# ribal-aladeeb/reinforcement-learning-2048

Hardware: AMD Instinct MI355X
Metric: 2048 env steps/sec + DQN updates/sec at 64k parallel boards, 1→8 MI355X (higher is better)
Workload: dtype u8

## Files before the change

reinforcement-learning-2048_amd/csrc/g2048_learn64.hip:

```cpp
#include <hip/hip_runtime.h>
#include <math.h>
#include <stdint.h>
#include <stdlib.h>

#include "../../include/g2048.h"
#include "g2048_board.hpp"
#include "g2048_common.hpp"

namespace {

constexpr int NT = 256;
constexpr int S = 64;
constexpr int XS = 17;
constexpr int HS = 65;
constexpr int P_W1 = 0, P_B1 = 1024, P_W2 = 1088, P_B2 = 1344, P_N = 1348;
constexpr int SLAB = P_N + 4;
constexpr int MAX_SLABS = 256;

struct Net64 {
    double *w1, *b1, *w2, *b2;
};

struct alignas(16) Smem {
    double x[S * XS];
    double h[S * HS];
    double w2[2][4 * 64];
    double b1[2][64];
    double b2[2][4];
    double qa[S * 4];
    double qb[S * 4];
    double y[S];
    double dq[S];
    double loss[S];
    int act[S];
};

__device__ __forceinline__ int64_t sample_row(int64_t b, unsigned long long ep,
                                              unsigned long long count, uint32_t lo, uint32_t hi) {
    const uint4 u = g2048::philox10(
        make_uint4((uint32_t)b, (uint32_t)((uint64_t)b >> 32), (uint32_t)ep,
                   (uint32_t)(ep >> 32) | (g2048::DOMAIN_SAMPLE << 30)),
        lo, hi);
    return (int64_t)__umul64hi(((unsigned long long)u.y << 32) | u.x, count);
}

__device__ __forceinline__ void put_row(double* xr, uint4 v) {
    const uint32_t w[4] = {v.x, v.y, v.z, v.w};
#pragma unroll
    for (int k = 0; k < 4; ++k) {
        xr[4 * k + 0] = (double)(w[k] & 0xFFu);
        xr[4 * k + 1] = (double)((w[k] >> 8) & 0xFFu);
        xr[4 * k + 2] = (double)((w[k] >> 16) & 0xFFu);
        xr[4 * k + 3] = (double)(w[k] >> 24);
    }
}

__device__ __forceinline__ void forward(Smem& M, const double (&w1r)[16], int net, double* q) {
    const int t = threadIdx.x, j = t & 63, rq = t >> 6;
    const double bj = M.b1[net][j];
#pragma unroll 4
    for (int rr = 0; rr < 16; ++rr) {
        const int s = rq * 16 + rr;
        const double* xr = M.x + s * XS;
        double acc = 0.0;
#pragma unroll
        for (int k = 0; k < 16; ++k) acc = fma(w1r[k], xr[k], acc);
        const double pre = acc + bj;
        M.h[s * HS + j] = pre > 0.0 ? pre : 0.0;
    }
    __syncthreads();
    const int s = t >> 2, a = t & 3;
    const double* hr = M.h + s * HS;
    const double* w2 = M.w2[net] + a * 64;
    double acc = 0.0;
#pragma unroll 8
    for (int jj = 0; jj < 64; ++jj) acc = fma(w2[jj], hr[jj], acc);
    q[s * 4 + a] = acc + M.b2[net][a];
    __syncthreads();
}

struct UpdArgs64 {
    Net64 on, tg;
    const uint4 *s, *s2;
    const uint8_t *a, *d;
    const int32_t* r;
    const unsigned long long* count;
    const unsigned long long* step;
    const int64_t* idx_in;
    int64_t batch;
    uint32_t seed_lo, seed_hi;
    float gamma;
    int double_dqn;
    int64_t* idx_out;
    double* y_out;
    double* slab;
    unsigned long long* step_next;
};

typedef uint32_t u32x2 __attribute__((ext_vector_type(2)));
constexpr int AUX_SC1 = 16;
__device__ __forceinline__ __amdgpu_buffer_rsrc_t slab_rsrc(const double* base) {
    return __builtin_amdgcn_make_buffer_rsrc(const_cast<double*>(base), 0, 0x7FFFFFFF, 0x00020000);
}
template <bool COH>
__device__ __forceinline__ void slab_put(double* sl, int e, double v) {
    if constexpr (COH)
        __builtin_amdgcn_raw_buffer_store_b64(__builtin_bit_cast(u32x2, v), slab_rsrc(sl),
                                              (uint32_t)e * 8u, 0u, AUX_SC1);
    else
        sl[e] = v;
}

template <bool COH>
__device__ __forceinline__ void update_tiles64(const UpdArgs64& A) {
    __shared__ Smem M;
    const int t = threadIdx.x, j = t & 63, qd = t >> 6;
    const unsigned long long ep = A.idx_in ? 0ull : *A.step;
    const unsigned long long count = A.idx_in ? 0ull : *A.count;
    if (blockIdx.x == 0 && t == 0) *A.step_next = *A.step + 1ull;
    const Net64 nets[2] = {A.tg, A.on};
    double w1t[16], w1o[16];
#pragma unroll
    for (int k = 0; k < 16; ++k) {
        w1t[k] = A.tg.w1[j * 16 + k];
        w1o[k] = A.on.w1[j * 16 + k];
    }
    for (int i = t; i < 2 * 256; i += NT) M.w2[i >> 8][i & 255] = nets[i >> 8].w2[i & 255];
    if (t < 128) M.b1[t >> 6][t & 63] = nets[t >> 6].b1[t & 63];
    if (t < 8) M.b2[t >> 2][t & 3] = nets[t >> 2].b2[t & 3];
    double w2o[4];
#pragma unroll
    for (int a = 0; a < 4; ++a) w2o[a] = A.on.w2[a * 64 + j];
    double g_w1[4] = {0.0, 0.0, 0.0, 0.0}, g_b1 = 0.0, g_w2 = 0.0, g_b2 = 0.0, g_loss = 0.0;
    const int64_t ntiles = (A.batch + S - 1) / S;
    for (int64_t tile = blockIdx.x; tile < ntiles; tile += gridDim.x) {
        const int64_t b = tile * S + t;
        uint4 sv = make_uint4(0u, 0u, 0u, 0u);
        double rj = 0.0;
        float disc = 0.f;
        bool ok = false;
        __syncthreads();
        if (t < S) {
            uint4 s2v = make_uint4(0u, 0u, 0u, 0u);
            int aj = 0;
            ok = b < A.batch;
            if (ok) {
                const int64_t row =
                    A.idx_in ? A.idx_in[b] : sample_row(b, ep, count, A.seed_lo, A.seed_hi);
                A.idx_out[b] = row;
                s2v = A.s2[row];
                sv = A.s[row];
                aj = A.a[row];
                rj = (double)A.r[row];
                disc = (float)(1 - (int)A.d[row]) * A.gamma;
            }
            put_row(M.x + t * XS, s2v);
            M.act[t] = aj;
        }
        __syncthreads();
        forward(M, w1t, 0, M.qa);
        forward(M, w1o, 1, M.qb);
        if (t < S) {
            const double* qo = M.qb + t * 4;
            const double* qt = M.qa + t * 4;
            double next;
            if (A.double_dqn) {
                const uint32_t as = g2048::argmax4_torch(qo[0], qo[1], qo[2], qo[3]);
                next = qt[as];
            } else {
                next = g2048::qmax4_torch(qt[0], qt[1], qt[2], qt[3]);
            }
            double y;
            {
#pragma clang fp contract(off)
                y = rj + (double)disc * next;
            }
            M.y[t] = y;
            if (ok) A.y_out[b] = y;
            put_row(M.x + t * XS, sv);
        }
        __syncthreads();
        forward(M, w1o, 1, M.qb);
        if (t < S) {
            double dq = 0.0, l = 0.0;
            if (ok) {
#pragma clang fp contract(off)
                const double e = M.qb[t * 4 + M.act[t]] - M.y[t];
                dq = 2.0 * e;
                l = e * e;
            }
            M.dq[t] = dq;
            M.loss[t] = l;
        }
        __syncthreads();
        {
            double acc = 0.0, accb = 0.0;
            for (int s = 0; s < S; ++s) {
                if (M.act[s] == qd) {
                    acc = fma(M.dq[s], M.h[s * HS + j], acc);
                    accb += M.dq[s];
                }
            }
            g_w2 += acc;
            if (j == 0) g_b2 += accb;
        }
        if (t == 0) {
            double l = 0.0;
            for (int s = 0; s < S; ++s) l += M.loss[s];
            g_loss += l;
        }
        __syncthreads();
#pragma unroll 4
        for (int rr = 0; rr < 16; ++rr) {
            const int s = qd * 16 + rr;
            double& hv = M.h[s * HS + j];
            const double w = M.act[s] == 0 ? w2o[0] : M.act[s] == 1 ? w2o[1]
                           : M.act[s] == 2 ? w2o[2] : w2o[3];
            hv = hv > 0.0 ? M.dq[s] * w : 0.0;
        }
        __syncthreads();
        {
            double acc[4] = {0.0, 0.0, 0.0, 0.0}, accb = 0.0;
            for (int s = 0; s < S; ++s) {
                const double dh = M.h[s * HS + j];
                const double* xr = M.x + s * XS + 4 * qd;
#pragma unroll
                for (int i = 0; i < 4; ++i) acc[i] = fma(dh, xr[i], acc[i]);
                accb += dh;
            }
#pragma unroll
            for (int i = 0; i < 4; ++i) g_w1[i] += acc[i];
            if (qd == 0) g_b1 += accb;
        }
    }
    double* sl = A.slab + (int64_t)blockIdx.x * SLAB;
#pragma unroll
    for (int i = 0; i < 4; ++i) slab_put<COH>(sl, P_W1 + j * 16 + 4 * qd + i, g_w1[i]);
    if (qd == 0) slab_put<COH>(sl, P_B1 + j, g_b1);
    slab_put<COH>(sl, P_W2 + qd * 64 + j, g_w2);
    if (j == 0) slab_put<COH>(sl, P_B2 + qd, g_b2);
    if (t == 0) slab_put<COH>(sl, P_N, g_loss);
}

__global__ __launch_bounds__(NT) void k_dense64_update_f64(UpdArgs64 A) { update_tiles64<false>(A); }

constexpr int RW = 16;
static_assert(MAX_SLABS <= RW * 16, "reduction covers at most RW*16 slabs");

struct RedArgs64 {
    const double* slab;
    int nslab;
    double* grad;
    double* loss;
    const unsigned long long* step_next;
    unsigned long long* step;
    double* p[4];
    double* tp[4];
    unsigned long long sync_every;
    double* m;
    double* v;
    double lr, b1, b2, eps;
    int adam;
};

template <int NW, bool COH>
__device__ __forceinline__ void reduce_positions64(const RedArgs64& A, int chunk,
                                                   unsigned long long t, double (*part)[64]) {
    const int lane = threadIdx.x & 63, wave = threadIdx.x >> 6;
    const int pos = chunk * 64 + lane;
    const int k = pos < P_B1 ? 0 : pos < P_W2 ? 1 : pos < P_B2 ? 2 : 3;
    const int base[4] = {P_W1, P_B1, P_W2, P_B2};
    const bool adam = A.adam && wave == 0 && pos < P_N;
    double am = 0.0, av = 0.0, ap = 0.0;
    if (adam) {
// ... 195 lines not shown
```

reinforcement-learning-2048_amd/csrc/g2048_mlp.hip:

```cpp
#include <hip/hip_runtime.h>
#include <stdint.h>
#include <stdlib.h>

#include "../../include/g2048.h"
#include "g2048_board.hpp"
#include "g2048_common.hpp"

namespace {

constexpr int NT = 256, H = 64;
constexpr int XS = 20, W1S = 17, HS = 68, W2S = 68;
constexpr int S_FWD = 64;
constexpr int S_UPD = 32;
constexpr int P_W1 = 0, P_B1 = 1024, P_W2 = 1088, P_B2 = 1344, P_N = 1348;
constexpr int SLAB = 1352;
constexpr int MAX_SLABS = 256;

struct MlpW {
    const float *w1, *b1, *w2, *b2;
};

struct alignas(16) LW {
    float w1[H * W1S];
    float b1[H];
    float w2[4 * W2S];
    float b2[4];
};

template <int S>
struct alignas(16) Tile {
    float x[S * XS];
    float h[S * HS];
    float q[S * 4];
    float a[S], y[S], g[S];
};

__device__ __forceinline__ void stage_weights(const MlpW& W, LW& L) {
    const int t = threadIdx.x;
#pragma unroll
    for (int u = 0; u < 4; ++u) {
        const int e = u * NT + t;
        L.w1[(e >> 4) * W1S + (e & 15)] = W.w1[e];
    }
    if (t < H) L.b1[t] = W.b1[t];
    L.w2[(t >> 6) * W2S + (t & 63)] = W.w2[t];
    if (t < 4) L.b2[t] = W.b2[t];
// ... 62 lines not shown
            }
            T.h[s * HS + j] = fmaxf((p[0] + p[1]) + (p[2] + p[3]), 0.f);
        }
    }
    __syncthreads();
    layer2_tile<S>(T, W);
}

typedef float f32x4m __attribute__((ext_vector_type(4)));

__device__ __forceinline__ float4 w1_lane(const MlpW& W) {
    const int lane = threadIdx.x & 63, wave = threadIdx.x >> 6;
    return reinterpret_cast<const float4*>(W.w1)[(16 * wave + (lane & 15)) * 4 + (lane >> 4)];
}

template <int S>
__device__ __forceinline__ void forward_tile_mfma(Tile<S>& T, const LW& W, float4 w1v) {
    const int lane = threadIdx.x & 63, wave = threadIdx.x >> 6, g = lane >> 4, l16 = lane & 15;
    const int j = 16 * wave + l16;
    const float bj = W.b1[j];
#pragma unroll
    for (int mb = 0; mb < S / 16; ++mb) {
        const float4 xv = *reinterpret_cast<const float4*>(T.x + (16 * mb + l16) * XS + 4 * g);
        f32x4m acc = {0.f, 0.f, 0.f, 0.f};
        acc = __builtin_amdgcn_mfma_f32_16x16x4f32(xv.x, w1v.x, acc, 0, 0, 0);
        acc = __builtin_amdgcn_mfma_f32_16x16x4f32(xv.y, w1v.y, acc, 0, 0, 0);
        acc = __builtin_amdgcn_mfma_f32_16x16x4f32(xv.z, w1v.z, acc, 0, 0, 0);
        acc = __builtin_amdgcn_mfma_f32_16x16x4f32(xv.w, w1v.w, acc, 0, 0, 0);
#pragma unroll
        for (int i = 0; i < 4; ++i) T.h[(16 * mb + 4 * g + i) * HS + j] = fmaxf(acc[i] + bj, 0.f);
    }
    __syncthreads();
    layer2_tile<S>(T, W);
}

__device__ __forceinline__ float bellman(const float* qo, const float* qt, int32_t r, uint8_t d,
                                         float gamma, int double_dqn) {
#pragma clang fp contract(off)
    float next;
    if (double_dqn) {
        next = qt[g2048::argmax4_torch(qo[0], qo[1], qo[2], qo[3])];
    } else {
        next = g2048::qmax4_torch(qt[0], qt[1], qt[2], qt[3]);
    }
    const float disc = (float)(1 - (int)d) * gamma;
    return (float)r + disc * next;
}

__device__ __forceinline__ int64_t sample_row(int64_t b, unsigned long long ep,
                                              unsigned long long count, uint32_t lo, uint32_t hi) {
    const uint4 u = g2048::philox10(
        make_uint4((uint32_t)b, (uint32_t)((uint64_t)b >> 32), (uint32_t)ep,
                   (uint32_t)(ep >> 32) | (g2048::DOMAIN_SAMPLE << 30)),
        lo, hi);
    return (int64_t)__umul64hi(((unsigned long long)u.y << 32) | u.x, count);
}

struct GradAcc {
    f32x4m w1a = {0.f, 0.f, 0.f, 0.f};
    f32x4m w1b = {0.f, 0.f, 0.f, 0.f};
    float b1 = 0.f, w2 = 0.f, b2 = 0.f, loss = 0.f;
};

template <int S>
__device__ __forceinline__ void grad_tile(Tile<S>& T, const LW& W, float4 w1v, GradAcc& G) {
    const int t = threadIdx.x;
    forward_tile_mfma<S>(T, W, w1v);
    if (t < S) {
        const float d = (T.q[t * 4 + (int)T.a[t]] - T.y[t]) * T.g[t];
        G.loss = fmaf(d, d, G.loss);
        T.g[t] = 2.f * d;
    }
    __syncthreads();
    {
        const int a = t >> 6, j = t & 63;
        float gw = 0.f, gb = 0.f;
#pragma unroll 8
        for (int s = 0; s < S; ++s) {
            const float g = (int)T.a[s] == a ? T.g[s] : 0.f;
            gw = fmaf(g, T.h[s * HS + j], gw);
            gb += g;
        }
        G.w2 += gw;
        if (j == 0) G.b2 += gb;
    }
    __syncthreads();
    {
        constexpr int SPT = S / 4;
// ... 69 lines not shown
    float* q;
};

__global__ __launch_bounds__(NT) void k_mlp_forward(FwdArgs A) {
    constexpr int S = S_FWD;
    __shared__ LW W;
    __shared__ Tile<S> T;
    const int64_t b0 = (int64_t)blockIdx.x * S;
    stage_weights(A.W, W);
    stage_boards<S>(T, A.rows, A.idx, b0, A.n);
    __syncthreads();
    forward_tile<S>(T, W);
    const int t = threadIdx.x;
    if (b0 + (t >> 2) < A.n) A.q[b0 * 4 + t] = T.q[t];
}

struct TargetArgs {
    MlpW on, tg;
    const uint8_t* s2;
    const int32_t* r;
    const uint8_t* d;
    const unsigned long long* count;
    const unsigned long long* epoch;
    const int64_t* idx_in;
    int64_t batch;
    uint32_t seed_lo, seed_hi;
    float gamma;
    int double_dqn;
    int64_t* idx_out;
    float* y;
};

__global__ __launch_bounds__(NT) void k_mlp_targets(TargetArgs A) {
    constexpr int S = S_FWD;
    __shared__ LW W;
    __shared__ Tile<S> T;
    __shared__ float qon[S * 4];
    __shared__ int64_t sidx[S];
    const int t = threadIdx.x;
    const int64_t b0 = (int64_t)blockIdx.x * S;
    if (t < S) {
        const int64_t b = b0 + t;
        int64_t j = 0;
        if (b < A.batch) {
            j = A.idx_in ? A.idx_in[b] : sample_row(b, *A.epoch, *A.count, A.seed_lo, A.seed_hi);
            A.idx_out[b] = j;
        }
        sidx[t] = j;
    }
    const float4 w1on = w1_lane(A.on), w1tg = w1_lane(A.tg);
    stage_weights(A.on, W);
    __syncthreads();
    stage_boards<S>(T, A.s2, sidx, 0, S);
    __syncthreads();
    forward_tile_mfma<S>(T, W, w1on);
    qon[t] = T.q[t];
    stage_weights(A.tg, W);
    __syncthreads();
    forward_tile_mfma<S>(T, W, w1tg);
    if (t < S && b0 + t < A.batch) {
        const int64_t j = sidx[t];
        A.y[b0 + t] = bellman(qon + t * 4, T.q + t * 4, A.r[j], A.d[j], A.gamma, A.double_dqn);
    }
}

struct TrainArgs {
    MlpW W;
    const uint8_t* rows;
    const uint8_t* actions;
    const int64_t* idx;
    const float* y;
    int64_t batch;
    float* slab;
    unsigned long long* step;
};

__global__ __launch_bounds__(NT) void k_mlp_train(TrainArgs A) {
    constexpr int S = S_FWD;
    __shared__ LW W;
    __shared__ Tile<S> T;
    const int t = threadIdx.x;
    if (A.step && blockIdx.x == 0 && t == 0) *A.step += 1ull;
    stage_weights(A.W, W);
    const float4 w1v = w1_lane(A.W);
    GradAcc G;
    const int64_t ntiles = (A.batch + S - 1) / S;
    for (int64_t tile = blockIdx.x; tile < ntiles; tile += gridDim.x) {
        const int64_t b0 = tile * S;
        __syncthreads();
        stage_boards<S>(T, A.rows, A.idx, b0, A.batch);
        if (t < S) {
            const int64_t b = b0 + t;
            const bool ok = b < A.batch;
            T.a[t] = ok ? (float)A.actions[A.idx[b]] : 0.f;
            T.y[t] = ok ? A.y[b] : 0.f;
            T.g[t] = ok ? 1.f : 0.f;
        }
        __syncthreads();
        grad_tile<S>(T, W, w1v, G);
    }
    write_slab<S>(G, T, A.slab + (int64_t)blockIdx.x * SLAB);
}

struct UpdateArgs {
    MlpW on, tg;
    const uint8_t *s, *a, *s2, *d;
    const int32_t* r;
    const unsigned long long* count;
    const unsigned long long* step;
    const int64_t* idx_in;
    int64_t batch;
    uint32_t seed_lo, seed_hi;
    float gamma;
    int double_dqn;
    int64_t* idx_out;
    float* y_out;
    float* slab;
    unsigned long long* step_next;
#ifdef G2048_MLP_PHASE
    long long* phase;
#endif
};

#ifdef G2048_MLP_PHASE
#define MPHASE(k) \
    if (threadIdx.x == 0) A.phase[blockIdx.x * 8 + (k)] = __builtin_amdgcn_s_memtime()
#else
#define MPHASE(k)
#endif

template <bool COH>
__device__ __forceinline__ void update_tiles(const UpdateArgs& A) {
    constexpr int S = S_UPD;
    MPHASE(0);
    __shared__ LW Won, Wtg;
    __shared__ Tile<S> T;
    __shared__ float qtg[S * 4];
    const int t = threadIdx.x;
    const unsigned long long ep = A.idx_in ? 0ull : *A.step;
    const unsigned long long count = A.idx_in ? 0ull : *A.count;
    if (blockIdx.x == 0 && t == 0) *A.step_next = *A.step + 1ull;
    stage_weights(A.on, Won);
    stage_weights(A.tg, Wtg);
    const float4 w1on = w1_lane(A.on), w1tg = w1_lane(A.tg);
    GradAcc G;
    const int64_t ntiles = (A.batch + S - 1) / S;
    const int sl = t >> 2, w = t & 3;
    for (int64_t tile = blockIdx.x; tile < ntiles; tile += gridDim.x) {
        const int64_t b0 = tile * S;
        const int64_t b = b0 + sl;
        const bool ok = t < 4 * S && b < A.batch;
        uint32_t s2w = 0, sw = 0;
        int32_t rj = 0;
        uint8_t dj = 0, aj = 0;
        if (ok) {
            const int64_t j =
                A.idx_in ? A.idx_in[b] : sample_row(b, ep, count, A.seed_lo, A.seed_hi);
            s2w = reinterpret_cast<const uint32_t*>(A.s2)[j * 4 + w];
            sw = reinterpret_cast<const uint32_t*>(A.s)[j * 4 + w];
            if (w == 0) {
                A.idx_out[b] = j;
                rj = A.r[j];
                dj = A.d[j];
                aj = A.a[j];
            }
        }
        __syncthreads();
        MPHASE(1);
        if (t < 4 * S) {
            put_word(T.x + sl * XS + w * 4, s2w);
            if (w == 0) {
                T.a[sl] = (float)aj;
                T.g[sl] = ok ? 1.f : 0.f;
            }
        }
        __syncthreads();
        MPHASE(2);
        forward_tile_mfma<S>(T, Wtg, w1tg);
        if (t < 4 * S) qtg[t] = T.q[t];
        forward_tile_mfma<S>(T, Won, w1on);
        if (t < 4 * S && w == 0) {
            const float y = bellman(T.q + sl * 4, qtg + sl * 4, rj, dj, A.gamma, A.double_dqn);
            T.y[sl] = y;
            if (ok) A.y_out[b] = y;
        }
        __syncthreads();
        MPHASE(3);
        if (t < 4 * S) put_word(T.x + sl * XS + w * 4, sw);
        __syncthreads();
        MPHASE(4);
        grad_tile<S>(T, Won, w1on, G);
#ifdef G2048_MLP_PHASE
        __syncthreads();
#endif
        MPHASE(5);
    }
    write_slab<S, COH>(G, T, A.slab + (int64_t)blockIdx.x * SLAB);
    MPHASE(6);
}

__global__ __launch_bounds__(NT) void k_mlp_update(UpdateArgs A) { update_tiles<false>(A); }

constexpr int RW = 16;
static_assert(MAX_SLABS <= RW * 16, "reduction covers at most RW*16 slabs");

struct ReduceArgs {
    const float* slab;
    int nslab;
    float* grad;
    float* loss;
    const unsigned long long* step_next;
    unsigned long long* step;
    float* p[4];
    float* tp[4];
    unsigned long long sync_every;
    float* m;
    float* v;
    double lr, b1, b2, eps;
    int adam;
};

template <int NW, bool COH>
__device__ __forceinline__ void reduce_positions(const ReduceArgs& A, int chunk,
                                                 unsigned long long t, float (*part)[64]) {
    const int lane = threadIdx.x & 63, wave = threadIdx.x >> 6;
    const int pos = chunk * 64 + lane;
    const bool adam = A.adam && wave == 0 && pos < P_N;
    const int k = pos < P_B1 ? 0 : pos < P_W2 ? 1 : pos < P_B2 ? 2 : 3;
    const int base[4] = {P_W1, P_B1, P_W2, P_B2};
    float am = 0.f, av = 0.f, ap = 0.f;
    if (adam) {
// ... 303 lines not shown
```

reinforcement-learning-2048_amd/g2048/qnet.py:

```python
from __future__ import annotations

import ctypes as C

import torch
from torch import nn

from . import _native as N
from .nets import Conv2048

_CONV_ORDER = ("0.weight", "0.bias", "2.weight", "2.bias", "5.weight", "5.bias", "7.weight",
               "7.bias")
_DENSE_ORDER = ("0.weight", "0.bias", "2.weight", "2.bias")


_DENSE_REF_ORDER = ("0.weight", "0.bias", "2.weight", "2.bias", "4.weight", "4.bias", "6.weight",
                    "6.bias")


def is_dense_ref(model) -> bool:
    dims = [(16, 512), (512, 512), (512, 256), (256, 4)]
    return (isinstance(model, nn.Sequential) and len(model) == 7
            and all(isinstance(model[2 * i], nn.Linear)
                    and (model[2 * i].in_features, model[2 * i].out_features) == d
                    for i, d in enumerate(dims))
# ... 283 lines not shown

    def reset_state(self):
        self.exp_avg.zero_()
        self.exp_avg_sq.zero_()

    def step(self, grad_flat: torch.Tensor, step_counter: torch.Tensor, grad_scale: float = 1.0):
        lib = N.load()
        args = (self._ptrs, self._numel, len(self.params), N.ptr(grad_flat), N.ptr(self.exp_avg),
                N.ptr(self.exp_avg_sq), N.ptr(step_counter), self.lr, self.betas[0], self.betas[1],
                self.eps, self._tptrs, self.sync_every if self._tptrs is not None else 0)
        if grad_scale == 1.0:
            N.check(lib.g2048_adam_step_sync_f64(*args, N.stream_of(grad_flat.device)),
                    "g2048_adam_step_sync_f64")
        else:
            N.check(lib.g2048_adam_step_scaled_f64(*args, float(grad_scale),
                                                   N.stream_of(grad_flat.device)),
                    "g2048_adam_step_scaled_f64")


class Dense64Update64:

    def __init__(self, model, target, batch: int, adam: Adam64 | None = None):
        if kind64_of(model) != "dense64" or kind64_of(target) != "dense64":
            raise TypeError("Dense64Update64 needs fp64 dense 16-64-4 online and target nets")
        self.on = N.Dense64Params(*[t.data_ptr() for t in
                                    _tensors(model, _DENSE_ORDER, torch.float64)])
        self.tg = N.Dense64Params(*[t.data_ptr() for t in
                                    _tensors(target, _DENSE_ORDER, torch.float64)])
        self.batch = int(batch)
        self.adam = adam
        dev = next(model.parameters()).device
        n = N.load().g2048_dense64_update_f64_workspace(self.batch)
        self.workspace = torch.zeros(n, dtype=torch.float64, device=dev)
        self._grid = min((self.batch + 63) // 64, 256)

    def sync_errors(self) -> int:
        return int(self.workspace[self._grid * 1352 + 1:].view(torch.int32)[2])

    def __call__(self, replay, idx_out, y_out, step_dev, gamma=0.8, double_dqn=True, seed=0,
                 idx_in=None, grad_out=None, loss_out=None):
        if idx_out.numel() != self.batch or y_out.numel() != self.batch:
            raise ValueError("idx_out / y_out must have `batch` elements")
        if y_out.dtype != torch.float64:
            raise TypeError("y_out must be float64")
        if self.adam is None and grad_out is None:
            raise ValueError("without Adam state the gradient needs a grad_out buffer")
        a = self.adam
        m, v = (a.exp_avg, a.exp_avg_sq) if a is not None else (None, None)
        lr, b1, b2, eps = (a.lr, a.betas[0], a.betas[1], a.eps) if a is not None else (0, 0, 0, 0)
        N.check(N.load().g2048_dense64_update_f64(
            C.byref(self.on), C.byref(self.tg), replay.handle, N.ptr(idx_in), self.batch,
            int(seed), N.ptr(step_dev), float(gamma), int(bool(double_dqn)), N.ptr(idx_out),
            N.ptr(y_out), N.ptr(self.workspace), N.ptr(grad_out), N.ptr(loss_out), N.ptr(m),
            N.ptr(v), float(lr), float(b1), float(b2), float(eps),
            int(a.sync_every) if a is not None else 0, N.stream_of(y_out.device)),
            "g2048_dense64_update_f64")


class ConvUpdate64:

    def __init__(self, model, target, batch: int, adam: Adam64 | None = None):
        if kind64_of(model) != "conv" or kind64_of(target) != "conv":
            raise TypeError("ConvUpdate64 needs fp64 Conv2048 online and target nets")
        self._params = (_tensors(model, _CONV_ORDER, torch.float64)
                        + _tensors(target, _CONV_ORDER, torch.float64))
        self.on = N.ConvNetParams(*[t.data_ptr() for t in self._params[:8]])
        self.tg = N.ConvNetParams(*[t.data_ptr() for t in self._params[8:]])
        self.batch = int(batch)
        self.adam = adam
        dev = next(model.parameters()).device
# ... 59 lines not shown
        self.workspace = torch.empty(n, dtype=dt, device=dev)

    def __call__(self, replay, idx_out, y_out, step_dev, gamma=0.8, double_dqn=True, seed=0,
                 idx_in=None, grad_out=None, loss_out=None):
        if idx_out.numel() != self.batch or y_out.numel() != self.batch:
            raise ValueError("idx_out / y_out must have `batch` elements")
        if y_out.dtype != self.dtype:
            raise TypeError(f"y_out must be {self.dtype}")
        if self.adam is None and grad_out is None:
            raise ValueError("without Adam state the gradient needs a grad_out buffer")
        a = self.adam
        m, v = (a.exp_avg, a.exp_avg_sq) if a is not None else (None, None)
        lr, b1, b2, eps = (a.lr, a.betas[0], a.betas[1], a.eps) if a is not None else (0, 0, 0, 0)
        N.check(N.load().g2048_densenet_update(
            C.byref(self.on), C.byref(self.tg), self.code, replay.handle, N.ptr(idx_in),
            self.batch, int(seed), N.ptr(step_dev), float(gamma), int(bool(double_dqn)),
            N.ptr(idx_out), N.ptr(y_out), N.ptr(self.workspace), N.ptr(grad_out),
            N.ptr(loss_out), N.ptr(m), N.ptr(v), float(lr), float(b1), float(b2), float(eps),
            int(a.sync_every) if a is not None else 0, N.stream_of(y_out.device)),
            "g2048_densenet_update")


class Dense64Update:

    def __init__(self, model, target, batch: int, adam=None):
        if kind_of(model) != "dense64" or kind_of(target) != "dense64":
            raise TypeError("Dense64Update needs fp32 dense 16-64-4 online and target nets")
        self.on, self.tg = net_params(model), net_params(target)
        self.batch = int(batch)
        self.adam = adam
        dev = next(model.parameters()).device
        n = N.load().g2048_dense64_update_workspace(self.batch)
        self.workspace = torch.zeros(n, dtype=torch.float32, device=dev)
        self._grid = min((self.batch + 31) // 32, 256)

    def sync_errors(self) -> int:
        tail = self.workspace[self._grid * 1352 + 2:].view(torch.int32)
        return int(tail[2])

    def __call__(self, replay, idx_out, y_out, step_dev, gamma=0.8, double_dqn=True, seed=0,
                 idx_in=None, grad_out=None, loss_out=None):
        if idx_out.numel() != self.batch or y_out.numel() != self.batch:
            raise ValueError("idx_out / y_out must have `batch` elements")
        if self.adam is None and grad_out is None:
            raise ValueError("without Adam state the gradient needs a grad_out buffer")
        a = self.adam
        m, v = (a.exp_avg, a.exp_avg_sq) if a is not None else (None, None)
        lr, b1, b2, eps = (a.lr, a.betas[0], a.betas[1], a.eps) if a is not None else (0, 0, 0, 0)
        N.check(N.load().g2048_dense64_update(
            C.byref(self.on), C.byref(self.tg), replay.handle, N.ptr(idx_in), self.batch,
            int(seed), N.ptr(step_dev), float(gamma), int(bool(double_dqn)), N.ptr(idx_out),
            N.ptr(y_out), N.ptr(self.workspace), N.ptr(grad_out), N.ptr(loss_out), N.ptr(m),
            N.ptr(v), float(lr), float(b1), float(b2), float(eps),
            int(a.sync_every) if a is not None else 0, N.stream_of(y_out.device)),
            "g2048_dense64_update")


def targets(kind: str, online, target, replay, batch: int, idx_out: torch.Tensor,
            y_out: torch.Tensor, gamma: float = 0.8, double_dqn: bool = True, seed: int = 0,
            epoch: torch.Tensor | None = None, idx_in: torch.Tensor | None = None):
    if idx_in is None and epoch is None:
        raise ValueError("need idx_in or a device epoch counter")
    N.check(_sym(kind, "targets")(
        C.byref(online), C.byref(target), replay.handle, N.ptr(idx_in), int(batch), int(seed),
        N.ptr(epoch), float(gamma), int(bool(double_dqn)), N.ptr(idx_out), N.ptr(y_out),
        N.stream_of(y_out.device)), "fused targets")
    return idx_out, y_out


def conv_targets(online, target, replay, batch, idx_out, y_out, gamma=0.8, double_dqn=True,
                 seed=0, epoch=None, idx_in=None):
# ... 3 lines not shown
```

Before: 170.9 billion.

## Rewrite dense64 DQN update as per-wave register MFMA kernels

```diff
diff --git a/reinforcement-learning-2048_amd/csrc/g2048_dense64_wave.hpp b/reinforcement-learning-2048_amd/csrc/g2048_dense64_wave.hpp
--- /dev/null
+++ b/reinforcement-learning-2048_amd/csrc/g2048_dense64_wave.hpp
@@ -0,0 +1,337 @@
+#pragma once
+#include <hip/hip_runtime.h>
+#include <stdint.h>
+
+#include "g2048_common.hpp"
+
+namespace g2048 {
+namespace wave16 {
+
+constexpr int H = 64;
+constexpr int P_W1 = 0, P_B1 = 1024, P_W2 = 1088, P_B2 = 1344, P_N = 1348;
+constexpr int ROWS = 16;
+
+template <typename T>
+struct Mx;
+template <>
+struct Mx<float> {
+    typedef float v4 __attribute__((ext_vector_type(4)));
+    static __device__ __forceinline__ v4 mfma(float a, float b, v4 c) {
+        return __builtin_amdgcn_mfma_f32_16x16x4f32(a, b, c, 0, 0, 0);
+    }
+    static __device__ __forceinline__ int row(int g, int i) { return 4 * g + i; }
+};
+template <>
+struct Mx<double> {
+    typedef double v4 __attribute__((ext_vector_type(4)));
+    static __device__ __forceinline__ v4 mfma(double a, double b, v4 c) {
+        return __builtin_amdgcn_mfma_f64_16x16x4f64(a, b, c, 0, 0, 0);
+    }
+    static __device__ __forceinline__ int row(int g, int i) { return g + 4 * i; }
+};
+
+__device__ __forceinline__ int64_t sample_row(int64_t b, unsigned long long ep,
+                                              unsigned long long count, uint32_t lo, uint32_t hi) {
+    const uint4 u = g2048::philox10(
+        make_uint4((uint32_t)b, (uint32_t)((uint64_t)b >> 32), (uint32_t)ep,
+                   (uint32_t)(ep >> 32) | (g2048::DOMAIN_SAMPLE << 30)),
+        lo, hi);
+    return (int64_t)__umul64hi(((unsigned long long)u.y << 32) | u.x, count);
+}
+
+template <typename T>
+__device__ __forceinline__ T pick4(const typename Mx<T>::v4& q, int a) {
+    return a == 0 ? q[0] : a == 1 ? q[1] : a == 2 ? q[2] : q[3];
+}
+
+template <typename T>
+__device__ __forceinline__ T target_y(const typename Mx<T>::v4& qo, const typename Mx<T>::v4& qt,
+                                      int32_t r, uint8_t d, float gamma, int double_dqn) {
+#pragma clang fp contract(off)
+    T next;
+    if (double_dqn) {
+        next = pick4<T>(qt, (int)g2048::argmax4_torch(qo[0], qo[1], qo[2], qo[3]));
+    } else {
+        next = g2048::qmax4_torch(qt[0], qt[1], qt[2], qt[3]);
+    }
+    const float disc = (float)(1 - (int)d) * gamma;
+    return (T)r + (T)disc * next;
+}
+
+template <typename T>
+struct NetRegs {
+    T w1[4][4];
+    T b1[4][4];
+    T w2a[4][4];
+    T b2[4];
+};
+
+template <typename T>
+__device__ __forceinline__ void load_net(NetRegs<T>& N, const T* w1, const T* b1, const T* w2,
+                                         const T* b2) {
+    const int lane = threadIdx.x & 63, g = lane >> 4, l16 = lane & 15;
+    int act = -1;
+#pragma unroll
+    for (int a = 0; a < 4; ++a)
+        if (l16 == Mx<T>::row(0, a)) act = a;
+#pragma unroll
+    for (int ub = 0; ub < 4; ++ub) {
+#pragma unroll
+        for (int u = 0; u < 4; ++u) N.w1[ub][u] = w1[(16 * ub + l16) * 16 + 4 * g + u];
+#pragma unroll
+        for (int i = 0; i < 4; ++i) {
+            const int unit = 16 * ub + Mx<T>::row(g, i);
+            N.b1[ub][i] = b1[unit];
+            const T w = w2[(act < 0 ? 0 : act) * H + unit];
+            N.w2a[ub][i] = act < 0 ? T(0) : w;
+        }
+    }
+#pragma unroll
+    for (int i = 0; i < 4; ++i) N.b2[i] = b2[i];
+}
+
+template <typename T>
+struct BwdRegs {
+    T b1s[4];
+    T w2g[4];
+};
+
+template <typename T>
+__device__ __forceinline__ void load_bwd(BwdRegs<T>& R, const T* b1, const T* w2) {
+    const int lane = threadIdx.x & 63, g = lane >> 4, l16 = lane & 15;
+#pragma unroll
+    for (int ub = 0; ub < 4; ++ub) {
+        R.b1s[ub] = b1[16 * ub + l16];
+        R.w2g[ub] = w2[g * H + 16 * ub + l16];
+    }
+}
+
+template <typename T>
+__device__ __forceinline__ void unpack(uint32_t v, T (&x)[4]) {
+    x[0] = (T)(v & 0xFFu);
+    x[1] = (T)((v >> 8) & 0xFFu);
+    x[2] = (T)((v >> 16) & 0xFFu);
+    x[3] = (T)(v >> 24);
+}
+
+template <typename T>
+__device__ __forceinline__ typename Mx<T>::v4 forward_q(const NetRegs<T>& N, const T (&x)[4]) {
+    typedef typename Mx<T>::v4 V4;
+    V4 h[4];
+#pragma unroll
+    for (int ub = 0; ub < 4; ++ub) {
+        V4 acc = {T(0), T(0), T(0), T(0)};
+#pragma unroll
+        for (int u = 0; u < 4; ++u) acc = Mx<T>::mfma(N.w1[ub][u], x[u], acc);
+#pragma unroll
+        for (int i = 0; i < 4; ++i) {
+            const T z = acc[i] + N.b1[ub][i];
+            h[ub][i] = z > T(0) ? z : T(0);
+        }
+    }
+    V4 qe = {T(0), T(0), T(0), T(0)}, qo = {T(0), T(0), T(0), T(0)};
+#pragma unroll
+    for (int ub = 0; ub < 4; ub += 2)
+#pragma unroll
+        for (int i = 0; i < 4; ++i) {
+            qe = Mx<T>::mfma(N.w2a[ub][i], h[ub][i], qe);
+            qo = Mx<T>::mfma(N.w2a[ub + 1][i], h[ub + 1][i], qo);
+        }
+    V4 q;
+#pragma unroll
+    for (int i = 0; i < 4; ++i) q[i] = (qe[i] + qo[i]) + N.b2[i];
+    return q;
+}
+
+template <typename T>
+struct Batch {
+    const uint32_t *s, *s2;
+    const uint8_t *a, *d;
+    const int32_t* r;
+    const int64_t* idx_in;
+    int64_t batch;
+    unsigned long long ep, count;
+    uint32_t seed_lo, seed_hi;
+    float gamma;
+    int double_dqn;
+    int64_t* idx_out;
+    T* y_out;
+};
+
+template <typename T>
+struct WaveGrad {
+    typedef typename Mx<T>::v4 V4;
+    V4 w1[4];
+    V4 w2[4];
+    T b1[4];
+    T b2;
+    T loss;
+    __device__ __forceinline__ WaveGrad() {
+#pragma unroll
+        for (int ub = 0; ub < 4; ++ub) {
+            w1[ub] = V4{T(0), T(0), T(0), T(0)};
+            w2[ub] = V4{T(0), T(0), T(0), T(0)};
+            b1[ub] = T(0);
+        }
+        b2 = T(0);
+        loss = T(0);
+    }
+};
+
+__device__ __forceinline__ float loss_dq(float qa, float y, float& loss) {
+    const float d = qa - y;
+    loss = fmaf(d, d, loss);
+    return 2.f * d;
+}
+__device__ __forceinline__ double loss_dq(double qa, double y, double& loss) {
+#pragma clang fp contract(off)
+    const double e = qa - y;
+    loss += e * e;
+    return 2.0 * e;
+}
+
+template <typename T>
+__device__ __forceinline__ void target_rows(const Batch<T>& B, const NetRegs<T>& on,
+                                            const NetRegs<T>& tg, int64_t b0) {
+    typedef typename Mx<T>::v4 V4;
+    const int lane = threadIdx.x & 63, g = lane >> 4, l16 = lane & 15;
+    const int64_t b = b0 + l16;
+    const bool ok = b < B.batch;
+    const int64_t bc = ok ? b : B.batch - 1;
+    const int64_t j =
+        B.idx_in ? B.idx_in[bc] : sample_row(bc, B.ep, B.count, B.seed_lo, B.seed_hi);
+    uint32_t s2w = B.s2[j * 4 + g];
+    int32_t rj = 0;
+    uint8_t dj = 0;
+    if (g == 0) {
+        rj = B.r[j];
+        dj = B.d[j];
+        if (ok) B.idx_out[b] = j;
+    }
+    if (!ok) s2w = 0u;
+    T x2[4];
+    unpack<T>(s2w, x2);
+    const V4 qt = forward_q<T>(tg, x2);
+    const V4 qo = forward_q<T>(on, x2);
+    if (g == 0 && ok) B.y_out[b] = target_y<T>(qo, qt, rj, dj, B.gamma, B.double_dqn);
+}
+
+struct NoPhase {
+    __device__ __forceinline__ void operator()(int) const {}
+};
+
+template <typename T, class Phase = NoPhase>
+__device__ __forceinline__ void update_rows(const Batch<T>& B, const NetRegs<T>& on,
+                                            const NetRegs<T>& tg, const BwdRegs<T>& bw,
+                                            int64_t b0, WaveGrad<T>& G, Phase ph = Phase()) {
+    typedef typename Mx<T>::v4 V4;
+    const int lane = threadIdx.x & 63, g = lane >> 4, l16 = lane & 15;
+    const int64_t b = b0 + l16;
+    const bool ok = b < B.batch;
+    const int64_t bc = ok ? b : B.batch - 1;
+    const int64_t j =
+        B.idx_in ? B.idx_in[bc] : sample_row(bc, B.ep, B.count, B.seed_lo, B.seed_hi);
+    uint32_t s2w = B.s2[j * 4 + g], sw = B.s[j * 4 + g];
+    int32_t rj = 0;
+    uint8_t dj = 0;
+    int aj = 0;
+    if (g == 0) {
+        rj = B.r[j];
+        dj = B.d[j];
+        aj = B.a[j];
+        if (ok) B.idx_out[b] = j;
+    }
+    if (!ok) s2w = sw = 0u;
+    T x2[4], x[4];
+    unpack<T>(s2w, x2);
+    unpack<T>(sw, x);
+    ph(1);
+    const V4 qt = forward_q<T>(tg, x2);
+    const V4 qo = forward_q<T>(on, x2);
+    T y = T(0);
+    if (g == 0) {
+        y = target_y<T>(qo, qt, rj, dj, B.gamma, B.double_dqn);
+        if (ok) B.y_out[b] = y;
+    }
+    ph(2);
+    const V4 q = forward_q<T>(on, x);
+    T dq = T(0);
+    if (g == 0 && ok) dq = loss_dq(pick4<T>(q, aj), y, G.loss);
+    ph(3);
+    T dqr[4];
+    int ar[4];
+    uint32_t xw[4];
+#pragma unroll
+    for (int i = 0; i < 4; ++i) {
+        const int src = Mx<T>::row(g, i);
+        dqr[i] = __shfl(dq, src, 64);
+        ar[i] = __shfl(aj, src, 64);
+        xw[i] = (uint32_t)__shfl((int)sw, 16 * (l16 >> 2) + src, 64);
+    }
+    V4 hs[4];
+#pragma unroll
+    for (int ub = 0; ub < 4; ++ub) {
+        V4 acc = {T(0), T(0), T(0), T(0)};
+#pragma unroll
+        for (int u = 0; u < 4; ++u) acc = Mx<T>::mfma(x[u], on.w1[ub][u], acc);
+#pragma unroll
+        for (int i = 0; i < 4; ++i) {
+            const T z = acc[i] + bw.b1s[ub];
+            hs[ub][i] = z > T(0) ? z : T(0);
+        }
+    }
+    T oh[4];
+#pragma unroll
+    for (int i = 0; i < 4; ++i) oh[i] = ar[i] == l16 ? dqr[i] : T(0);
+#pragma unroll
+    for (int i = 0; i < 4; ++i)
+#pragma unroll
+        for (int ub = 0; ub < 4; ++ub) G.w2[ub] = Mx<T>::mfma(hs[ub][i], oh[i], G.w2[ub]);
+    G.b2 += ((oh[0] + oh[1]) + oh[2]) + oh[3];
+    const int a16 = __shfl(aj, l16, 64);
+    const T dq16 = __shfl(dq, l16, 64);
+    const T oha = a16 == g ? dq16 : T(0);
+    T xt[4];
+#pragma unroll
+    for (int i = 0; i < 4; ++i) xt[i] = (T)((xw[i] >> (8 * (l16 & 3))) & 0xFFu);
+#pragma unroll
+    for (int ub = 0; ub < 4; ++ub) {
+        const V4 dqw = Mx<T>::mfma(oha, bw.w2g[ub], V4{T(0), T(0), T(0), T(0)});
+        T dh[4];
+#pragma unroll
+        for (int i = 0; i < 4; ++i) dh[i] = hs[ub][i] > T(0) ? dqw[i] : T(0);
+#pragma unroll
+        for (int i = 0; i < 4; ++i) G.w1[ub] = Mx<T>::mfma(dh[i], xt[i], G.w1[ub]);
+        G.b1[ub] += ((dh[0] + dh[1]) + dh[2]) + dh[3];
+    }
+    ph(4);
+}
+
+template <typename T>
+__device__ __forceinline__ void put_image(const WaveGrad<T>& G, T* sm) {
+    const int lane = threadIdx.x & 63, g = lane >> 4, l16 = lane & 15;
+#pragma unroll
+    for (int ub = 0; ub < 4; ++ub) {
+#pragma unroll
+        for (int i = 0; i < 4; ++i) {
+            const int unit = 16 * ub + Mx<T>::row(g, i);
+            sm[P_W1 + unit * 16 + l16] = G.w1[ub][i];
+            if (l16 < 4) sm[P_W2 + l16 * H + unit] = G.w2[ub][i];
+        }
+        T v = G.b1[ub];
+        v += __shfl_xor(v, 16, 64);
+        v += __shfl_xor(v, 32, 64);
+        if (g == 0) sm[P_B1 + 16 * ub + l16] = v;
+    }
+    T v = G.b2;
+    v += __shfl_xor(v, 16, 64);
+    v += __shfl_xor(v, 32, 64);
+    if (g == 0 && l16 < 4) sm[P_B2 + l16] = v;
+    T l = G.loss;
+#pragma unroll
+    for (int m = 1; m < 16; m <<= 1) l += __shfl_xor(l, m, 64);
+    if (lane == 0) sm[P_N] = l;
+}
+
+}
+}
diff --git a/reinforcement-learning-2048_amd/csrc/g2048_learn64.hip b/reinforcement-learning-2048_amd/csrc/g2048_learn64.hip
--- a/reinforcement-learning-2048_amd/csrc/g2048_learn64.hip
+++ b/reinforcement-learning-2048_amd/csrc/g2048_learn64.hip
@@ -6,78 +6,23 @@
 #include "../../include/g2048.h"
 #include "g2048_board.hpp"
 #include "g2048_common.hpp"
+#include "g2048_dense64_wave.hpp"
 
 namespace {
 
 constexpr int NT = 256;
 constexpr int S = 64;
-constexpr int XS = 17;
-constexpr int HS = 65;
-constexpr int P_W1 = 0, P_B1 = 1024, P_W2 = 1088, P_B2 = 1344, P_N = 1348;
+using g2048::wave16::P_B1;
+using g2048::wave16::P_B2;
+using g2048::wave16::P_N;
+using g2048::wave16::P_W1;
+using g2048::wave16::P_W2;
 constexpr int SLAB = P_N + 4;
 constexpr int MAX_SLABS = 256;
 
 struct Net64 {
     double *w1, *b1, *w2, *b2;
 };
-
-struct alignas(16) Smem {
-    double x[S * XS];
-    double h[S * HS];
-    double w2[2][4 * 64];
-    double b1[2][64];
-    double b2[2][4];
-    double qa[S * 4];
-    double qb[S * 4];
-    double y[S];
-    double dq[S];
-    double loss[S];
-    int act[S];
-};
-
-__device__ __forceinline__ int64_t sample_row(int64_t b, unsigned long long ep,
-                                              unsigned long long count, uint32_t lo, uint32_t hi) {
-    const uint4 u = g2048::philox10(
-        make_uint4((uint32_t)b, (uint32_t)((uint64_t)b >> 32), (uint32_t)ep,
-                   (uint32_t)(ep >> 32) | (g2048::DOMAIN_SAMPLE << 30)),
-        lo, hi);
-    return (int64_t)__umul64hi(((unsigned long long)u.y << 32) | u.x, count);
-}
-
-__device__ __forceinline__ void put_row(double* xr, uint4 v) {
-    const uint32_t w[4] = {v.x, v.y, v.z, v.w};
-#pragma unroll
-    for (int k = 0; k < 4; ++k) {
-        xr[4 * k + 0] = (double)(w[k] & 0xFFu);
-        xr[4 * k + 1] = (double)((w[k] >> 8) & 0xFFu);
-        xr[4 * k + 2] = (double)((w[k] >> 16) & 0xFFu);
-        xr[4 * k + 3] = (double)(w[k] >> 24);
-    }
-}
-
-__device__ __forceinline__ void forward(Smem& M, const double (&w1r)[16], int net, double* q) {
-    const int t = threadIdx.x, j = t & 63, rq = t >> 6;
-    const double bj = M.b1[net][j];
-#pragma unroll 4
-    for (int rr = 0; rr < 16; ++rr) {
-        const int s = rq * 16 + rr;
-        const double* xr = M.x + s * XS;
-        double acc = 0.0;
-#pragma unroll
-        for (int k = 0; k < 16; ++k) acc = fma(w1r[k], xr[k], acc);
-        const double pre = acc + bj;
-        M.h[s * HS + j] = pre > 0.0 ? pre : 0.0;
-    }
-    __syncthreads();
-    const int s = t >> 2, a = t & 3;
-    const double* hr = M.h + s * HS;
-    const double* w2 = M.w2[net] + a * 64;
-    double acc = 0.0;
-#pragma unroll 8
-    for (int jj = 0; jj < 64; ++jj) acc = fma(w2[jj], hr[jj], acc);
-    q[s * 4 + a] = acc + M.b2[net][a];
-    __syncthreads();
-}
 
 struct UpdArgs64 {
     Net64 on, tg;
@@ -113,133 +58,49 @@
 
 template <bool COH>
 __device__ __forceinline__ void update_tiles64(const UpdArgs64& A) {
-    __shared__ Smem M;
-    const int t = threadIdx.x, j = t & 63, qd = t >> 6;
-    const unsigned long long ep = A.idx_in ? 0ull : *A.step;
-    const unsigned long long count = A.idx_in ? 0ull : *A.count;
+    namespace W = g2048::wave16;
+    __shared__ double img[NT / 64][SLAB];
+    const int t = threadIdx.x, wave = t >> 6;
+    W::Batch<double> B;
+    B.s = reinterpret_cast<const uint32_t*>(A.s);
+    B.s2 = reinterpret_cast<const uint32_t*>(A.s2);
+    B.a = A.a;
+    B.d = A.d;
+    B.r = A.r;
+    B.idx_in = A.idx_in;
+    B.batch = A.batch;
+    B.ep = A.idx_in ? 0ull : *A.step;
+    B.count = A.idx_in ? 0ull : *A.count;
+    B.seed_lo = A.seed_lo;
+    B.seed_hi = A.seed_hi;
+    B.gamma = A.gamma;
+    B.double_dqn = A.double_dqn;
+    B.idx_out = A.idx_out;
+    B.y_out = A.y_out;
     if (blockIdx.x == 0 && t == 0) *A.step_next = *A.step + 1ull;
-    const Net64 nets[2] = {A.tg, A.on};
-    double w1t[16], w1o[16];
-#pragma unroll
-    for (int k = 0; k < 16; ++k) {
-        w1t[k] = A.tg.w1[j * 16 + k];
-        w1o[k] = A.on.w1[j * 16 + k];
-    }
-    for (int i = t; i < 2 * 256; i += NT) M.w2[i >> 8][i & 255] = nets[i >> 8].w2[i & 255];
-    if (t < 128) M.b1[t >> 6][t & 63] = nets[t >> 6].b1[t & 63];
-    if (t < 8) M.b2[t >> 2][t & 3] = nets[t >> 2].b2[t & 3];
-    double w2o[4];
-#pragma unroll
-    for (int a = 0; a < 4; ++a) w2o[a] = A.on.w2[a * 64 + j];
-    double g_w1[4] = {0.0, 0.0, 0.0, 0.0}, g_b1 = 0.0, g_w2 = 0.0, g_b2 = 0.0, g_loss = 0.0;
+    W::NetRegs<double> on, tg;
+    W::BwdRegs<double> bw;
+    W::load_net<double>(tg, A.tg.w1, A.tg.b1, A.tg.w2, A.tg.b2);
+    W::load_net<double>(on, A.on.w1, A.on.b1, A.on.w2, A.on.b2);
+    W::load_bwd<double>(bw, A.on.b1, A.on.w2);
+    W::WaveGrad<double> G;
     const int64_t ntiles = (A.batch + S - 1) / S;
     for (int64_t tile = blockIdx.x; tile < ntiles; tile += gridDim.x) {
-        const int64_t b = tile * S + t;
-        uint4 sv = make_uint4(0u, 0u, 0u, 0u);
-        double rj = 0.0;
-        float disc = 0.f;
-        bool ok = false;
-        __syncthreads();
-        if (t < S) {
-            uint4 s2v = make_uint4(0u, 0u, 0u, 0u);
-            int aj = 0;
-            ok = b < A.batch;
-            if (ok) {
-                const int64_t row =
-                    A.idx_in ? A.idx_in[b] : sample_row(b, ep, count, A.seed_lo, A.seed_hi);
-                A.idx_out[b] = row;
-                s2v = A.s2[row];
-                sv = A.s[row];
-                aj = A.a[row];
-                rj = (double)A.r[row];
-                disc = (float)(1 - (int)A.d[row]) * A.gamma;
-            }
-            put_row(M.x + t * XS, s2v);
-            M.act[t] = aj;
-        }
-        __syncthreads();
-        forward(M, w1t, 0, M.qa);
-        forward(M, w1o, 1, M.qb);
-        if (t < S) {
-            const double* qo = M.qb + t * 4;
-            const double* qt = M.qa + t * 4;
-            double next;
-            if (A.double_dqn) {
-                const uint32_t as = g2048::argmax4_torch(qo[0], qo[1], qo[2], qo[3]);
-                next = qt[as];
-            } else {
-                next = g2048::qmax4_torch(qt[0], qt[1], qt[2], qt[3]);
-            }
-            double y;
-            {
-#pragma clang fp contract(off)
-                y = rj + (double)disc * next;
-            }
-            M.y[t] = y;
-            if (ok) A.y_out[b] = y;
-            put_row(M.x + t * XS, sv);
-        }
-        __syncthreads();
-        forward(M, w1o, 1, M.qb);
-        if (t < S) {
-            double dq = 0.0, l = 0.0;
-            if (ok) {
-#pragma clang fp contract(off)
-                const double e = M.qb[t * 4 + M.act[t]] - M.y[t];
-                dq = 2.0 * e;
-                l = e * e;
-            }
-            M.dq[t] = dq;
-            M.loss[t] = l;
-        }
-        __syncthreads();
-        {
-            double acc = 0.0, accb = 0.0;
-            for (int s = 0; s < S; ++s) {
-                if (M.act[s] == qd) {
-                    acc = fma(M.dq[s], M.h[s * HS + j], acc);
-                    accb += M.dq[s];
-                }
-            }
-            g_w2 += acc;
-            if (j == 0) g_b2 += accb;
-        }
-        if (t == 0) {
-            double l = 0.0;
-            for (int s = 0; s < S; ++s) l += M.loss[s];
-            g_loss += l;
-        }
-        __syncthreads();
-#pragma unroll 4
-        for (int rr = 0; rr < 16; ++rr) {
-            const int s = qd * 16 + rr;
-            double& hv = M.h[s * HS + j];
-            const double w = M.act[s] == 0 ? w2o[0] : M.act[s] == 1 ? w2o[1]
-                           : M.act[s] == 2 ? w2o[2] : w2o[3];
-            hv = hv > 0.0 ? M.dq[s] * w : 0.0;
-        }
-        __syncthreads();
-        {
-            double acc[4] = {0.0, 0.0, 0.0, 0.0}, accb = 0.0;
-            for (int s = 0; s < S; ++s) {
-                const double dh = M.h[s * HS + j];
-                const double* xr = M.x + s * XS + 4 * qd;
-#pragma unroll
-                for (int i = 0; i < 4; ++i) acc[i] = fma(dh, xr[i], acc[i]);
-                accb += dh;
-            }
-#pragma unroll
-            for (int i = 0; i < 4; ++i) g_w1[i] += acc[i];
-            if (qd == 0) g_b1 += accb;
-        }
-    }
+        const int64_t b0 = tile * S + W::ROWS * wave;
+        if (b0 < A.batch) W::update_rows<double>(B, on, tg, bw, b0, G);
+    }
+    W::put_image<double>(G, img[wave]);
+    __syncthreads();
     double* sl = A.slab + (int64_t)blockIdx.x * SLAB;
-#pragma unroll
-    for (int i = 0; i < 4; ++i) slab_put<COH>(sl, P_W1 + j * 16 + 4 * qd + i, g_w1[i]);
-    if (qd == 0) slab_put<COH>(sl, P_B1 + j, g_b1);
-    slab_put<COH>(sl, P_W2 + qd * 64 + j, g_w2);
-    if (j == 0) slab_put<COH>(sl, P_B2 + qd, g_b2);
-    if (t == 0) slab_put<COH>(sl, P_N, g_loss);
+    double sum[(P_N + NT) / NT];
+#pragma unroll
+    for (int k = 0; k < (P_N + NT) / NT; ++k) {
+        const int p = t + k * NT < P_N ? t + k * NT : P_N;
+        sum[k] = ((img[0][p] + img[1][p]) + img[2][p]) + img[3][p];
+    }
+#pragma unroll
+    for (int k = 0; k < (P_N + NT) / NT; ++k)
+        if (t + k * NT <= P_N) slab_put<COH>(sl, t + k * NT, sum[k]);
 }
 
 __global__ __launch_bounds__(NT) void k_dense64_update_f64(UpdArgs64 A) { update_tiles64<false>(A); }
diff --git a/reinforcement-learning-2048_amd/csrc/g2048_mlp.hip b/reinforcement-learning-2048_amd/csrc/g2048_mlp.hip
--- a/reinforcement-learning-2048_amd/csrc/g2048_mlp.hip
+++ b/reinforcement-learning-2048_amd/csrc/g2048_mlp.hip
@@ -5,13 +5,14 @@
 #include "../../include/g2048.h"
 #include "g2048_board.hpp"
 #include "g2048_common.hpp"
+#include "g2048_dense64_wave.hpp"
 
 namespace {
 
 constexpr int NT = 256, H = 64;
 constexpr int XS = 20, W1S = 17, HS = 68, W2S = 68;
 constexpr int S_FWD = 64;
-constexpr int S_UPD = 32;
+constexpr int S_UPD = 64;
 constexpr int P_W1 = 0, P_B1 = 1024, P_W2 = 1088, P_B2 = 1344, P_N = 1348;
 constexpr int SLAB = 1352;
 constexpr int MAX_SLABS = 256;
@@ -140,28 +141,6 @@
     }
     __syncthreads();
     layer2_tile<S>(T, W);
-}
-
-__device__ __forceinline__ float bellman(const float* qo, const float* qt, int32_t r, uint8_t d,
-                                         float gamma, int double_dqn) {
-#pragma clang fp contract(off)
-    float next;
-    if (double_dqn) {
-        next = qt[g2048::argmax4_torch(qo[0], qo[1], qo[2], qo[3])];
-    } else {
-        next = g2048::qmax4_torch(qt[0], qt[1], qt[2], qt[3]);
-    }
-    const float disc = (float)(1 - (int)d) * gamma;
-    return (float)r + disc * next;
-}
-
-__device__ __forceinline__ int64_t sample_row(int64_t b, unsigned long long ep,
-                                              unsigned long long count, uint32_t lo, uint32_t hi) {
-    const uint4 u = g2048::philox10(
-        make_uint4((uint32_t)b, (uint32_t)((uint64_t)b >> 32), (uint32_t)ep,
-                   (uint32_t)(ep >> 32) | (g2048::DOMAIN_SAMPLE << 30)),
-        lo, hi);
-    return (int64_t)__umul64hi(((unsigned long long)u.y << 32) | u.x, count);
 }
 
 struct GradAcc {
@@ -297,36 +276,27 @@
 };
 
 __global__ __launch_bounds__(NT) void k_mlp_targets(TargetArgs A) {
-    constexpr int S = S_FWD;
-    __shared__ LW W;
-    __shared__ Tile<S> T;
-    __shared__ float qon[S * 4];
-    __shared__ int64_t sidx[S];
-    const int t = threadIdx.x;
-    const int64_t b0 = (int64_t)blockIdx.x * S;
-    if (t < S) {
-        const int64_t b = b0 + t;
-        int64_t j = 0;
-        if (b < A.batch) {
-            j = A.idx_in ? A.idx_in[b] : sample_row(b, *A.epoch, *A.count, A.seed_lo, A.seed_hi);
-            A.idx_out[b] = j;
-        }
-        sidx[t] = j;
-    }
-    const float4 w1on = w1_lane(A.on), w1tg = w1_lane(A.tg);
-    stage_weights(A.on, W);
-    __syncthreads();
-    stage_boards<S>(T, A.s2, sidx, 0, S);
-    __syncthreads();
-    forward_tile_mfma<S>(T, W, w1on);
-    qon[t] = T.q[t];
-    stage_weights(A.tg, W);
-    __syncthreads();
-    forward_tile_mfma<S>(T, W, w1tg);
-    if (t < S && b0 + t < A.batch) {
-        const int64_t j = sidx[t];
-        A.y[b0 + t] = bellman(qon + t * 4, T.q + t * 4, A.r[j], A.d[j], A.gamma, A.double_dqn);
-    }
+    namespace W = g2048::wave16;
+    const int64_t b0 = (int64_t)blockIdx.x * S_FWD + W::ROWS * (threadIdx.x >> 6);
+    if (b0 >= A.batch) return;
+    W::Batch<float> B{};
+    B.s2 = reinterpret_cast<const uint32_t*>(A.s2);
+    B.d = A.d;
+    B.r = A.r;
+    B.idx_in = A.idx_in;
+    B.batch = A.batch;
+    B.ep = A.idx_in ? 0ull : *A.epoch;
+    B.count = A.idx_in ? 0ull : *A.count;
+    B.seed_lo = A.seed_lo;
+    B.seed_hi = A.seed_hi;
+    B.gamma = A.gamma;
+    B.double_dqn = A.double_dqn;
+    B.idx_out = A.idx_out;
+    B.y_out = A.y;
+    W::NetRegs<float> on, tg;
+    W::load_net<float>(tg, A.tg.w1, A.tg.b1, A.tg.w2, A.tg.b2);
+    W::load_net<float>(on, A.on.w1, A.on.b1, A.on.w2, A.on.b2);
+    W::target_rows<float>(B, on, tg, b0);
 }
 
 struct TrainArgs {
@@ -387,81 +357,73 @@
 #endif
 };
 
+struct MlpPhase {
 #ifdef G2048_MLP_PHASE
-#define MPHASE(k) \
-    if (threadIdx.x == 0) A.phase[blockIdx.x * 8 + (k)] = __builtin_amdgcn_s_memtime()
+    long long* p;
+    __device__ __forceinline__ void operator()(int k) const {
+        __builtin_amdgcn_s_waitcnt(0);
+        __builtin_amdgcn_sched_barrier(0);
+        if (threadIdx.x == 0) p[blockIdx.x * 8 + k] = __builtin_amdgcn_s_memtime();
+        __builtin_amdgcn_sched_barrier(0);
+    }
 #else
-#define MPHASE(k)
+    __device__ __forceinline__ void operator()(int) const {}
 #endif
+};
 
 template <bool COH>
 __device__ __forceinline__ void update_tiles(const UpdateArgs& A) {
+    namespace W = g2048::wave16;
     constexpr int S = S_UPD;
-    MPHASE(0);
-    __shared__ LW Won, Wtg;
-    __shared__ Tile<S> T;
-    __shared__ float qtg[S * 4];
-    const int t = threadIdx.x;
-    const unsigned long long ep = A.idx_in ? 0ull : *A.step;
-    const unsigned long long count = A.idx_in ? 0ull : *A.count;
+    __shared__ float img[NT / 64][SLAB];
+    const int t = threadIdx.x, wave = t >> 6;
+#ifdef G2048_MLP_PHASE
+    const MlpPhase ph{A.phase};
+#else
+    const MlpPhase ph{};
+#endif
+    ph(0);
+    W::Batch<float> B;
+    B.s = reinterpret_cast<const uint32_t*>(A.s);
+    B.s2 = reinterpret_cast<const uint32_t*>(A.s2);
+    B.a = A.a;
+    B.d = A.d;
+    B.r = A.r;
+    B.idx_in = A.idx_in;
+    B.batch = A.batch;
+    B.ep = A.idx_in ? 0ull : *A.step;
+    B.count = A.idx_in ? 0ull : *A.count;
+    B.seed_lo = A.seed_lo;
+    B.seed_hi = A.seed_hi;
+    B.gamma = A.gamma;
+    B.double_dqn = A.double_dqn;
+    B.idx_out = A.idx_out;
+    B.y_out = A.y_out;
     if (blockIdx.x == 0 && t == 0) *A.step_next = *A.step + 1ull;
-    stage_weights(A.on, Won);
-    stage_weights(A.tg, Wtg);
-    const float4 w1on = w1_lane(A.on), w1tg = w1_lane(A.tg);
-    GradAcc G;
+    W::NetRegs<float> on, tg;
+    W::BwdRegs<float> bw;
+    W::load_net<float>(tg, A.tg.w1, A.tg.b1, A.tg.w2, A.tg.b2);
+    W::load_net<float>(on, A.on.w1, A.on.b1, A.on.w2, A.on.b2);
+    W::load_bwd<float>(bw, A.on.b1, A.on.w2);
+    W::WaveGrad<float> G;
     const int64_t ntiles = (A.batch + S - 1) / S;
-    const int sl = t >> 2, w = t & 3;
     for (int64_t tile = blockIdx.x; tile < ntiles; tile += gridDim.x) {
-        const int64_t b0 = tile * S;
-        const int64_t b = b0 + sl;
-        const bool ok = t < 4 * S && b < A.batch;
-        uint32_t s2w = 0, sw = 0;
-        int32_t rj = 0;
-        uint8_t dj = 0, aj = 0;
-        if (ok) {
-            const int64_t j =
-                A.idx_in ? A.idx_in[b] : sample_row(b, ep, count, A.seed_lo, A.seed_hi);
-            s2w = reinterpret_cast<const uint32_t*>(A.s2)[j * 4 + w];
-            sw = reinterpret_cast<const uint32_t*>(A.s)[j * 4 + w];
-            if (w == 0) {
-                A.idx_out[b] = j;
-                rj = A.r[j];
-                dj = A.d[j];
-                aj = A.a[j];
-            }
-        }
-        __syncthreads();
-        MPHASE(1);
-        if (t < 4 * S) {
-            put_word(T.x + sl * XS + w * 4, s2w);
-            if (w == 0) {
-                T.a[sl] = (float)aj;
-                T.g[sl] = ok ? 1.f : 0.f;
-            }
-        }
-        __syncthreads();
-        MPHASE(2);
-        forward_tile_mfma<S>(T, Wtg, w1tg);
-        if (t < 4 * S) qtg[t] = T.q[t];
-        forward_tile_mfma<S>(T, Won, w1on);
-        if (t < 4 * S && w == 0) {
-            const float y = bellman(T.q + sl * 4, qtg + sl * 4, rj, dj, A.gamma, A.double_dqn);
-            T.y[sl] = y;
-            if (ok) A.y_out[b] = y;
-        }
-        __syncthreads();
-        MPHASE(3);
-        if (t < 4 * S) put_word(T.x + sl * XS + w * 4, sw);
-        __syncthreads();
-        MPHASE(4);
-        grad_tile<S>(T, Won, w1on, G);
-#ifdef G2048_MLP_PHASE
-        __syncthreads();
-#endif
-        MPHASE(5);
-    }
-    write_slab<S, COH>(G, T, A.slab + (int64_t)blockIdx.x * SLAB);
-    MPHASE(6);
+        const int64_t b0 = tile * S + W::ROWS * wave;
+        if (b0 < A.batch) W::update_rows<float>(B, on, tg, bw, b0, G, ph);
+    }
+    W::put_image<float>(G, img[wave]);
+    __syncthreads();
+    float* slab = A.slab + (int64_t)blockIdx.x * SLAB;
+    float sum[(P_N + NT) / NT];
+#pragma unroll
+    for (int k = 0; k < (P_N + NT) / NT; ++k) {
+        const int p = t + k * NT < P_N ? t + k * NT : P_N;
+        sum[k] = ((img[0][p] + img[1][p]) + img[2][p]) + img[3][p];
+    }
+#pragma unroll
+    for (int k = 0; k < (P_N + NT) / NT; ++k)
+        if (t + k * NT <= P_N) slab_put<COH>(slab, t + k * NT, sum[k]);
+    ph(5);
 }
 
 __global__ __launch_bounds__(NT) void k_mlp_update(UpdateArgs A) { update_tiles<false>(A); }
diff --git a/reinforcement-learning-2048_amd/g2048/qnet.py b/reinforcement-learning-2048_amd/g2048/qnet.py
--- a/reinforcement-learning-2048_amd/g2048/qnet.py
+++ b/reinforcement-learning-2048_amd/g2048/qnet.py
@@ -339,10 +339,10 @@
         dev = next(model.parameters()).device
         n = N.load().g2048_dense64_update_f64_workspace(self.batch)
         self.workspace = torch.zeros(n, dtype=torch.float64, device=dev)
-        self._grid = min((self.batch + 63) // 64, 256)
+        self._grid = n // 1352
 
     def sync_errors(self) -> int:
-        return int(self.workspace[self._grid * 1352 + 1:].view(torch.int32)[2])
+        return int(self.workspace.view(torch.int32)[-2])
 
     def __call__(self, replay, idx_out, y_out, step_dev, gamma=0.8, double_dqn=True, seed=0,
                  idx_in=None, grad_out=None, loss_out=None):
@@ -468,11 +468,10 @@
         dev = next(model.parameters()).device
         n = N.load().g2048_dense64_update_workspace(self.batch)
         self.workspace = torch.zeros(n, dtype=torch.float32, device=dev)
-        self._grid = min((self.batch + 31) // 32, 256)
+        self._grid = n // 1352
 
     def sync_errors(self) -> int:
-        tail = self.workspace[self._grid * 1352 + 2:].view(torch.int32)
-        return int(tail[2])
+        return int(self.workspace.view(torch.int32)[-2])
 
     def __call__(self, replay, idx_out, y_out, step_dev, gamma=0.8, double_dqn=True, seed=0,
                  idx_in=None, grad_out=None, loss_out=None):
```

New measurement: 171.1 billion (median of 3 runs). No clear change (+0.1%).
